# djeedai/bevy_hanabi

Hardware: AMD Instinct MI355X
Metric: particle-updates/sec (higher is better)
Workload: dtype f32

## Files before the change

### bevy_hanabi_amd/build.py

```python
import os
import subprocess
import sys
import sysconfig

_DIR = os.path.dirname(os.path.abspath(__file__))
_CSRC = os.path.join(_DIR, "csrc")

HIP_FLAGS = ["--offload-arch=gfx950", "-O3", "-std=c++17", "-ffp-contract=off", "-fhip-fp32-correctly-rounded-divide-sqrt",
             "-fPIC", "-shared", "-Wno-unused-value"]
HOST_FLAGS = ["-std=c++17", "-O2", "-fPIC", "-shared", "-ffp-contract=off", "-fvisibility=hidden"]


def _newer(target, sources):
    if not os.path.exists(target):
        return True
    t = os.path.getmtime(target)
    return any(os.path.getmtime(s) > t for s in sources)


def runtime_lib_path():
    return os.path.join(_DIR, "libhanabi_amd.so")


def host_module_path():
# ... 123 lines not shown
    return _build_code_object("hnb_import", "kImportCode", ["-ffp-contract=off"], force, verbose, headers=("hnb_import.h", "hnb_export.h", "hnb_export_rows.hip.h", "hnb_sort_key.h"))


IMPORT_CODE_OBJECTS = (build_import_code,)


def build_bounds_code(force=False, verbose=False):
    return _build_code_object("hnb_bounds", "kBoundsCode", ["-ffp-contract=off"], force, verbose, headers=("hnb_bounds.h", "hnb_sort_key.h"))


QUERY_CODE_OBJECTS = (build_bounds_code,)


def build_runtime(force=False, verbose=False):
    srcs = [os.path.join(_CSRC, "hanabi_amd.hip")] + sorted(os.path.join(_CSRC, f) for f in os.listdir(_CSRC) if f.endswith(".h"))
    srcs += [os.path.join(_DIR, "..", "include", h) for h in ("hanabi_amd.h", "hanabi_amd_binned.h", "hanabi_amd_import.h")]
    for build_code in EXPORT_CODE_OBJECTS + BINNED_CODE_OBJECTS + IMPORT_CODE_OBJECTS + QUERY_CODE_OBJECTS:
        srcs.append(build_code(force, verbose))
    out = runtime_lib_path()
    if force or _newer(out, srcs):
        embed_headers()
        hipcc = os.environ.get("HIPCC", "/opt/rocm/bin/hipcc")
        cmd = [hipcc] + HIP_FLAGS + [srcs[0], "-o", out, "-lhiprtc", "-ldl"]
        if verbose:
            print(" ".join(cmd))
        subprocess.check_call(cmd, cwd=_CSRC)
    return out


def build_host(force=False, verbose=False):
    import pybind11
# ... 63 lines not shown
```

### bevy_hanabi_amd/csrc/hanabi_amd.hip

```cpp
#include <hip/hip_runtime.h>

#include <algorithm>
#include <atomic>
#include <chrono>
#include <cmath>
#include <condition_variable>
#include <cstdarg>
#include <cstdio>
#include <cstring>
#include <deque>
#include <memory>
#include <mutex>
#include <string>
#include <thread>
#include <vector>

#include "hnb_kernels.hip.h"
#include "hnb_jit.h"
#include "hnb_sort.hip.h"
#include "hnb_comm.h"
#include "hnb_plan.h"
#include "hnb_program.h"
#include "hnb_export.h"
#include "hnb_export_code.inc"
#include "hnb_export_sort_code.inc"
#include "hnb_filter_pred.h"
#include "hnb_export_filter_code.inc"
#include "hnb_export_cull_code.inc"
#include "hnb_export_filter_prog_code.inc"
#include "hnb_export_cull_prog_code.inc"
#include "hnb_export_bin.h"
#include "hnb_export_bin_code.inc"
#include "hnb_import.h"
#include "hnb_import_code.inc"
#include "hnb_bounds.h"
#include "hnb_bounds_code.inc"

using namespace hnb;

namespace {

thread_local std::string g_last_error;

int fail(int code, const char* fmt, ...) {
    char buf[512];
    va_list ap;
    va_start(ap, fmt);
    vsnprintf(buf, sizeof buf, fmt, ap);
    va_end(ap);
    g_last_error = buf;
// ... 138 lines not shown
    bool direct_failed = false;
    uint64_t direct_frames = 0, copied_frames = 0;
    uint64_t ring_waits = 0, ring_wait_ns = 0;
    hipEvent_t stage_done[plan::kStageGroups] = {};
    plan::StageRing stage_ring;
    uint32_t num_cus = 256;
    std::vector<HnbProgram*> programs;
    HnbSimParams sim{};
    uint32_t frame = 0;
    uint32_t list_order = HNB_LIST_ORDER_SPAWN;
    ProgramOptions popt;
    bool skip_lists = true;
    bool alternate = true;
    bool suffix_proof = true;
    uint32_t slot_init = 1;
    bool ring_lists = true;
    bool scene_merge = true;
    bool transpose = true;
    uint32_t timing = 0;
    uint32_t timing_tick = 0;
    std::vector<TimingPair> t_update, t_init, t_compact;
    std::vector<hipEvent_t> event_pool;
    uint32_t comm_refs = 0;
    uint32_t set_mode = HNB_SET_MODULE_CACHED;
    struct SetModule {
        hipModule_t module = nullptr;
        hipFunction_t init = nullptr, update = nullptr;
        jit::SetPlan plan;
        uint32_t gen = 0;
    } set;
// ... 29 lines not shown
    uint32_t cull_dt_operand = 0;
    bool update_streams = false;
    uint32_t age_cohort_mode = HNB_AGE_COHORT_AUTO;
    bool auto_materialise = false;
    StreamLaunchFn stream_launch = nullptr;
    StreamLaunchFn stream_launch_fused = nullptr;
    uint32_t fuse_span = 1, fused_left = 0;
    uint32_t safe_launches = 0;
    std::vector<uint32_t> fuse_ublocks;
    uint32_t fused_frames = 0;
    const char* stream_kernel_name = "";
    hipModule_t jit_module = nullptr;
    hipFunction_t jit_init = nullptr, jit_update = nullptr, jit_init_slots = nullptr;
    bool slot_init_eligible = false;
    uint32_t slot_init_frames = 0;
    uint32_t sort_skipped_frames = 0;
    uint32_t sort_path_frames[3] = {0, 0, 0};
    bool tick_sign_seen = false;
    uint64_t serial = 0;
    bool jit_pending = false;
    std::string kernel_info, jit_log;
    enum class StepsState { NotRequested, Built, Pending, Failed };
    hipModule_t steps_module = nullptr;
    hipFunction_t steps_update = nullptr;
    StepsState steps_state = StepsState::NotRequested;
    bool steps_from_cache = false;
    std::string steps_why;
    std::vector<Ins> steps_ops;
    int steps_waves = 0;
    bool steps_cohort = false;
// ... 527 lines not shown
        case HNB_OPT_HORIZON: ctx->popt.horizon = value != 0u; return HNB_OK;
        case HNB_OPT_TEST_BREAK_PROOF: {
            const char* e = getenv("HNB_ENABLE_TEST_HOOKS");
            if (value != 0u && !(e && e[0] == '1')) return fail(HNB_ERR_INVALID_ARG, "HNB_OPT_TEST_BREAK_PROOF is a test hook: refused unless HNB_ENABLE_TEST_HOOKS=1 is set in the environment");
            ctx->break_proof = value != 0u;
            return HNB_OK;
        }
        case HNB_OPT_TRANSPOSE: ctx->transpose = value != 0u; return HNB_OK;
        case HNB_OPT_SCENE_MERGE: ctx->scene_merge = value != 0u; return HNB_OK;
        case HNB_OPT_SUFFIX_PROOF: ctx->suffix_proof = value != 0u; return HNB_OK;
        case HNB_OPT_RING_LISTS: ctx->ring_lists = value != 0u; return HNB_OK;
        case HNB_OPT_SLOT_INIT:
            if (value > 2u) return fail(HNB_ERR_INVALID_ARG, "unknown slot-init mode %u", value);
            ctx->slot_init = value;
            return HNB_OK;
        case HNB_OPT_STREAM_HINTS: ctx->stream_hints = value != 0u; return HNB_OK;
        case HNB_OPT_DIRECT_UPLOAD: ctx->direct_upload = value != 0u; return HNB_OK;
        case HNB_OPT_JIT_ASYNC: ctx->jit_async = value != 0u; return HNB_OK;
        case HNB_OPT_FUSE_STEPS: ctx->fuse_steps = value != 0u; return HNB_OK;
        case HNB_OPT_SET_MODULE:
            if (value > HNB_SET_MODULE_BACKGROUND) return fail(HNB_ERR_INVALID_ARG, "unknown set-module mode %u", value);
            ctx->set_mode = value;
            ctx->set_lookup = plan::SetLookupState();
            return HNB_OK;
        case HNB_OPT_OVERLAP_UPDATES: ctx->overlap_updates = value != 0u && ctx->side_stream && ctx->ev_fork && ctx->ev_join; return HNB_OK;
        default: return fail(HNB_ERR_INVALID_ARG, "unknown option %u", option);
    }
}

int hnb_ctx_synchronize(HnbContext* ctx) {
// ... 1031 lines not shown
        const uint32_t grid = split ? total_chunks * (kChunk / kBlock) : total_chunks;
        ctx->step_stats.update_launches += 1;
        if (p->jit_update) {
            uint32_t dm = write_died;
            void* ka[] = {&p->dev, &p->d_inst_base, &dfi, &dub, &cb, &dm, &split};
            HIP_TRY(hipModuleLaunchKernel(p->jit_update, grid, 1, 1, kBlock, 1, 1, 0, st, ka, nullptr));
        } else if (p->wide_file) k_update_slots_generic<InterpCodeWide><<<grid, kBlock, 0, st>>>(p->dev, p->d_inst_base, dfi, dub, cb, write_died, split);
        else k_update_slots_generic<InterpCode><<<grid, kBlock, 0, st>>>(p->dev, p->d_inst_base, dfi, dub, cb, write_died, split);
    }
    if (timed) { hipEventRecord(tu.b, st); ctx->t_update.push_back(tu); }
    const CompactArgs ca = compact_args_of(p);
    const bool lists = p->plan.lists;
    if (!lists) p->skipped_frames += p->fuse_span;
    else if (ca.suffix_dead) p->suffix_frames += 1;
    if (lists && p->dev.n_event_channels) {
        k_emit_count<<<total_chunks, kBlock, 0, st>>>(p->dev, p->d_inst_base, p->d_meta[par], dfi, cb);
        uint32_t max_ev = 0;
        for (const HnbEffect* fx : p->effects)
            for (const EventChannel& ch : fx->channels) max_ev = std::max(max_ev, ch.capacity);
        const uint32_t splits = plan::size_event_grid(max_ev, total_chunks);
        k_emit_events<<<dim3(total_chunks, splits), kBlock, 0, st>>>(p->dev, p->d_inst_base, p->d_meta[par], dfi, cb, p->h_ev_counts, ctx->frame);
    }
    if (!p->plan.lists_merged) {
        if (lists) ctx->step_stats.list_launches += ((!p->slot_order && !ca.suffix_dead) ? 2u : 1u) + (p->slot_order ? 2u : 0u);
        if (lists && !p->slot_order && !ca.suffix_dead) k_count_rows<<<total_chunks, kBlock, 0, st>>>(ca, p->d_inst_base, p->d_meta[par], dfi, cb);
        if (lists) k_compact<<<total_chunks, kBlock, 0, st>>>(ca, p->d_inst_base, p->d_meta[par], p->d_meta[par ^ 1], dfi, cb);
        if (lists && p->slot_order) {
            k_order_count<<<total_chunks, kBlock, 0, st>>>(ca, p->d_inst_base, p->d_meta[par], dfi, cb);
            k_order_write<<<total_chunks, kBlock, 0, st>>>(ca, p->d_inst_base, p->d_meta[par], p->d_meta[par ^ 1], dfi, cb);
        }
        if (timed) { tc.a = tu.b; hipEventRecord(tc.b, st); ctx->t_compact.push_back(tc); }
        if (p->has_ribbons) enqueue_ribbon_sort(ctx, p, st);
    }
    HIP_TRY(hipGetLastError());
    return HNB_OK;
}
// ... 925 lines not shown
        if (l.step == kImportStepMaterialise) { if ((rc = enqueue_export_materialise(p, fx->index, 1u)) != HNB_OK) return rc; }
        else if (l.step == kImportStepZeroCounts) HIP_TRY(hipMemsetAsync(d->out_count, 0, 8u, ctx->stream));
        else {
            void* ka[] = {&a};
            HIP_TRY(hipModuleLaunchKernel(ctx->import_fn[l.kernel], l.grid_x, 1, 1, kExportBlock, 1, 1, 0, ctx->stream, ka, nullptr));
        }
    }
    if (c.n_payload == 0u) return HNB_OK;
    return reset_plane_proofs(fx, c.has_age);
}
}

int hnb_effect_import(HnbEffect* fx, const HnbImportDesc* desc) {
    if (!fx || !desc) return fail(HNB_ERR_INVALID_ARG, "NULL argument");
    return run_import(fx, desc);
}

int hnb_program_export(HnbProgram* p, const HnbExportDesc* desc, uint32_t* out_offsets) {
    if (!p || !desc) return fail(HNB_ERR_INVALID_ARG, "NULL argument");
    return run_export(p, nullptr, desc, nullptr, nullptr, HNB_SORT_SCOPE_INSTANCE, out_offsets);
}

int hnb_program_export_sorted(HnbProgram* p, const HnbExportDesc* desc, const HnbExportSort* sort, uint32_t scope, uint32_t* out_offsets) {
    if (!p || !desc || !sort) return fail(HNB_ERR_INVALID_ARG, "NULL argument");
    if (scope > HNB_SORT_SCOPE_PROGRAM) return fail(HNB_ERR_INVALID_ARG, "scope %u: HNB_SORT_SCOPE_INSTANCE or HNB_SORT_SCOPE_PROGRAM", scope);
    if (scope == HNB_SORT_SCOPE_PROGRAM && out_offsets)
        return fail(HNB_ERR_INVALID_ARG, "out_offsets must be NULL with HNB_SORT_SCOPE_PROGRAM: the records are one order over all instances (tell them apart by an HNB_ATTR_ID field)");
    if (sort->struct_size == sizeof(HnbExportSortFiltered)) {
        if (scope == HNB_SORT_SCOPE_PROGRAM)
            return fail(HNB_ERR_INVALID_ARG, "an HnbExportSortFiltered takes HNB_SORT_SCOPE_INSTANCE: one order over all instances' kept rows (HNB_SORT_SCOPE_PROGRAM) is out of scope");
// ... 245 lines not shown
    }
    if (!prog->dev.age_cohort && prog->dev.cull_lifetime && prog->age_cohort_mode == HNB_AGE_COHORT_AUTO && (prog->hdr.render_reads_lo >> HNB_ATTR_AGE & 1u))
        s += "\nage cohorts: off (HNB_AGE_COHORT_AUTO: the asset's render modifiers read AGE after every frame)";
    if (prog->dev.age_cohort) {
        hipStreamSynchronize(prog->ctx->stream);
        std::vector<uint32_t> st(prog->dev.chunks_per_inst);
        size_t in_cohort = 0;
        for (const HnbEffect* fx : prog->effects) {
            if (hipMemcpy(st.data(), static_cast<const char*>(fx->slab) + prog->dev.lmin_off + (size_t)prog->dev.chunks_per_inst * 8, st.size() * 4, hipMemcpyDeviceToHost) != hipSuccess) break;
            for (uint32_t v : st) in_cohort += v == 1u ? 1u : 0u;
        }
        s += "\nage cohorts: " + std::to_string(in_cohort) + " of " + std::to_string(prog->effects.size() * (size_t)prog->dev.chunks_per_inst) + " chunks";
        if (prog->auto_materialise) s += " (HNB_AGE_COHORT_AUTO: the asset's render modifiers read AGE, the update keeps the plane current)";
    }
    if (prog->slot_init_frames) s += "\nslot-major init (large spawns): " + std::to_string(prog->slot_init_frames) + " frames";
    if (prog->has_ribbons && prog->suffix_frames) s += "\ncasualties proven to be the list's last rows (no k_count_rows): " + std::to_string(prog->suffix_frames) + " frames";
    if (prog->has_ribbons && prog->ring_frames) s += "\nlist kept as a ring (no row rewritten): " + std::to_string(prog->ring_frames) + " frames";
    if (prog->has_ribbons && prog->sort_skipped_frames) s += "\nribbon sorts skipped in list-free frames: " + std::to_string(prog->sort_skipped_frames) + " frames";
    if (prog->has_ribbons) s += "\nribbon sorts by rotation: " + std::to_string(prog->sort_rotated_frames) + " of " + std::to_string(prog->frames_run) + " frames" + (prog->ribbon_facts.front_static ? "" : " (not eligible)");
    if (prog->has_ribbons) s += "\nribbon sorts by path: one-tile " + std::to_string(prog->sort_path_frames[0]) + ", one-workgroup " + std::to_string(prog->sort_path_frames[1]) +
                                ", multi-launch " + std::to_string(prog->sort_path_frames[2]) + " frames";
    if (prog->merged_frames) s += "\nupdate served by a merged launch (small programs of the context share one): " + std::to_string(prog->merged_frames) + " frames";
    if (prog->unmerged_frames) s += "\nkept out of the shared launches (the loaded set module does not know this program; its own specialised kernels): " + std::to_string(prog->unmerged_frames) + " frames";
    if (prog->set_frames) s += "\n... by the context's set module (the program's specialised code behind the shared launch): " + std::to_string(prog->set_frames) + " frames";
    if (!prog->ctx->set_log.empty() && !prog->set_sig.empty()) s += "\nset module: " + prog->ctx->set_log;
    if (prog->ctx->set_failed_builds && !prog->set_sig.empty()) s += "\nset module builds that failed: " + std::to_string(prog->ctx->set_failed_builds);
    if (prog->horizon_eligible) s += "\ndeath horizons in use: " + std::to_string(prog->hz_frames) + " frames";
    s += "\nlists skipped: " + std::to_string(prog->skipped_frames) + " of " + std::to_string(prog->frames_run) + " frames" + (prog->skip_facts.eligible ? "" : " (not eligible)");
    s += "\nframe parameters (context): written by the host into device memory in " + std::to_string(prog->ctx->direct_frames) + " frames, copied in " + std::to_string(prog->ctx->copied_frames) +
         (prog->ctx->large_bar ? "" : " (the device memory is not host-visible: no large BAR)") + (prog->ctx->direct_failed ? " (host-visible slots failed their check)" : "");
// ... 270 lines not shown
```

### bevy_hanabi_amd/csrc/hnb_kernels.hip.h

```cpp
#pragma once
#ifndef __HIPCC_RTC__
#include <hip/hip_runtime.h>
#endif
#include "hnb_dev.h"

namespace hnb {

template <class T>
__device__ __forceinline__ T* global_ptr(uint64_t addr) {
    typedef __attribute__((address_space(1))) T global_t;
    return (T*)(global_t*)addr;
}

struct u2_t { uint32_t x, y; };
struct u3_t { uint32_t x, y, z; };
typedef uint32_t u4v __attribute__((ext_vector_type(4)));
#if defined(HNB_NONTEMPORAL) || defined(HNB_NONTEMPORAL_LOADS)
#define HNB_NT_LOAD(p) __builtin_nontemporal_load(p)
#else
#define HNB_NT_LOAD(p) (*(p))
#endif
#if defined(HNB_NONTEMPORAL) || defined(HNB_NONTEMPORAL_STORES)
#define HNB_NT_STORE(v, p) __builtin_nontemporal_store(v, p)
#else
// ... 875 lines not shown
        if (slot >= args.capacity) break;
        if (mask & (1u << b)) s_alive[pos++] = slot;
        else s_free[fpos++] = slot;
    }
    __syncthreads();
    uint32_t* list = reinterpret_cast<uint32_t*>(c.base + args.alive_off[meta_out[c.k].write_index & 1u]) + excl;
    for (uint32_t i = tid; i < chunk_alive; i += kBlock) list[i] = s_alive[i];
    const uint32_t alive_total = meta_out[c.k].alive_count;
    uint32_t* dead = reinterpret_cast<uint32_t*>(c.base + args.dead_off) + alive_total + (chunk_first - excl);
    for (uint32_t i = tid; i < chunk_slots - chunk_alive; i += kBlock) dead[i] = s_free[i];
}
#endif

#ifndef HNB_JIT_TU
constexpr uint32_t kEmitHeavy = 32u;
__global__ void __launch_bounds__(kBlock)
k_emit_events(const DevProgram prog, const uint64_t* __restrict__ inst_base, const DevMeta* __restrict__ meta_in,
              const DevFrameInst* __restrict__ fi, const CompactBufs cb, unsigned long long* __restrict__ ev_host, const uint32_t frame_tag) {
    __shared__ uint32_t s_red[kBlock / 64];
    __shared__ uint32_t s_scan[kBlock / 64];
    __shared__ uint32_t s_heavy_n;
    __shared__ uint32_t s_heavy[kChunk][3];
    const uint32_t tid = threadIdx.x, lane = tid & 63u, wave = tid >> 6;
    const uint32_t chunk = chunk_of_workgroup(cb.xcd_remap);
    const uint32_t split = blockIdx.y, n_split = gridDim.y;
    ChunkCtx c;
    const bool has_rows = chunk_setup(c, chunk, prog, inst_base, meta_in, fi);
    const bool last = c.n == 0 ? c.j == 0 : (c.start < c.n && c.start + kChunk >= c.n);
    const uint32_t rows = has_rows ? ((c.n - c.start) < kChunk ? (c.n - c.start) : kChunk) : 0u;
    constexpr uint32_t kPer = kChunk / kBlock;
    for (uint32_t ch = 0; ch < prog.n_event_channels; ++ch) {
        DevEventBuffer* ev = global_ptr<DevEventBuffer>(fi[c.k].ev_out[ch]);
        if (!ev) continue;
        const uint32_t* tot = cb.ev_totals + (size_t)c.k * prog.chunks_per_inst * HNB_MAX_EVENT_CHANNELS + ch;
        uint32_t part = 0;
        for (uint32_t i = tid; i < c.j; i += kBlock) part += tot[(size_t)i * HNB_MAX_EVENT_CHANNELS];
#pragma unroll
        for (uint32_t off = 32; off > 0; off >>= 1) part += __shfl_xor(part, off, 64);
        __syncthreads();
        if (lane == 0) s_red[wave] = part;
        if (tid == 0) s_heavy_n = 0u;
        __syncthreads();
        uint32_t excl = 0;
#pragma unroll
        for (uint32_t w = 0; w < kBlock / 64; ++w) excl += s_red[w];
        const uint32_t mine = has_rows ? tot[(size_t)c.j * HNB_MAX_EVENT_CHANNELS] : 0u;
        if (last && tid == 0 && split == 0u) {
            ev->count[fi[c.k].ev_parity] = excl + mine;
            if (ev_host) *reinterpret_cast<volatile unsigned long long*>(ev_host + (size_t)c.k * HNB_MAX_EVENT_CHANNELS + ch) = ((unsigned long long)(excl + mine) << 32) | frame_tag;
        }
        const uint32_t capacity = ev->capacity;
        if (mine == 0u || excl >= capacity) continue;
        const uint32_t* cnt = reinterpret_cast<const uint32_t*>(c.base + prog.ev_cnt_off[ch]);
        const uint32_t* slots = reinterpret_cast<const uint32_t*>(c.base + prog.alive_off[list_column(c.m.write_index)]) + c.start;
        uint32_t slot[kPer], n_ev[kPer], local = 0;
#pragma unroll
        for (uint32_t r = 0; r < kPer; ++r) {
            const uint32_t row = tid * kPer + r;
            slot[r] = row < rows ? slots[row] : 0u;
            n_ev[r] = row < rows ? cnt[slot[r]] : 0u;
            local += n_ev[r];
        }
        uint32_t incl = local;
#pragma unroll
        for (uint32_t off = 1; off < 64; off <<= 1) { const uint32_t y = __shfl_up(incl, off, 64); if (lane >= off) incl += y; }
        if (lane == 63) s_scan[wave] = incl;
        __syncthreads();
        uint32_t pos = excl + incl - local;
        for (uint32_t w = 0; w < wave; ++w) pos += s_scan[w];
#pragma unroll
        for (uint32_t r = 0; r < kPer; ++r) {
            if (n_ev[r] >= kEmitHeavy) {
                if ((tid * kPer + r) % n_split == split) {
                    const uint32_t h = atomicAdd(&s_heavy_n, 1u);
                    s_heavy[h][0] = slot[r]; s_heavy[h][1] = pos; s_heavy[h][2] = n_ev[r];
                }
            } else if (split == 0u) {
                const uint32_t end = pos + n_ev[r] < capacity ? pos + n_ev[r] : capacity;
                for (uint32_t e = pos; e < end; ++e) ev->data[e] = slot[r];
            }
            pos += n_ev[r];
        }
        __syncthreads();
        const uint32_t n_heavy = s_heavy_n;
        for (uint32_t h = 0; h < n_heavy; ++h) {
            const uint32_t sl = s_heavy[h][0], first = s_heavy[h][1];
            const uint32_t end = first + s_heavy[h][2] < capacity ? first + s_heavy[h][2] : capacity;
            for (uint32_t e = first + tid; e < end; e += kBlock) ev->data[e] = sl;
        }
        __syncthreads();
    }
}
#endif

#ifndef HNB_STREAM_WAVES
#define HNB_STREAM_WAVES 6
#endif
#ifndef HNB_STREAM_WAVES_FULL
#define HNB_STREAM_WAVES_FULL 5
#endif

template <bool B> struct BoolTag { static constexpr bool value = B; };
struct SlotArgs {
    uint32_t capacity, n_uregs, chunks_per_inst, n_inst;
    soff_t alive_flag_off;
    uint32_t update_len;
// ... 891 lines not shown
```

### bevy_hanabi_amd/csrc/hnb_plan.h

```cpp
#pragma once
#include <cstdint>
#include <cstring>

namespace hnb {
namespace plan {

struct InstanceFrame {
    bool simulated = true;
    bool has_parent = false;
    uint32_t spawn_count = 0;
    uint32_t event_capacity = 0;
    const uint32_t* ublock = nullptr;
};
inline uint32_t uword(const InstanceFrame& f, uint32_t decoded_operand) { return f.ublock[decoded_operand & 0xffu]; }
inline float as_float(uint32_t bits) { float f; std::memcpy(&f, &bits, 4); return f; }
inline bool nonneg_not_nan(uint32_t float_bits) { return float_bits <= 0x7f800000u; }

struct SkipFacts {
    bool eligible = false;
    uint32_t dt_operand = 0;
};
struct SkipHistory {
    double cum_tick[128] = {};
    uint32_t last_dirty = 0;
// ... 143 lines not shown
    if (in.has_parent && in.simulated) {
        request = in.event_capacity;
        if (in.events_known) request = in.known_events < in.event_capacity ? in.known_events : in.event_capacity;
    }
    const uint32_t capped = request < capacity ? request : capacity;
    uint32_t blocks = (uint32_t)(((uint64_t)capped + init_block - 1u) / init_block);
    if (big_burst) blocks = (blocks + rounds_if_big - 1u) / rounds_if_big;
    if (in.has_parent) blocks = blocks < num_cus * 8u ? blocks : num_cus * 8u;
    return blocks;
}
inline uint32_t size_event_grid(uint32_t max_event_capacity, uint32_t total_chunks) {
    const uint32_t per_chunk = max_event_capacity / (total_chunks ? total_chunks : 1u);
    const uint32_t splits = (per_chunk + 16383u) / 16384u;
    return splits < 1u ? 1u : (splits > 64u ? 64u : splits);
}

struct SlotInitDecision { bool use = false, marks = false; };
constexpr uint32_t kSlotInitMinChunks = 17;
inline SlotInitDecision plan_slot_init(bool eligible, uint32_t option, uint32_t capacity, uint32_t chunks_per_inst, const InstanceFrame* inst, uint32_t n) {
    SlotInitDecision d;
    if (!eligible || option == 0u || n == 0u || (option == 1u && (uint64_t)n * chunks_per_inst < kSlotInitMinChunks)) return d;
    uint64_t spawns = 0;
    bool partial = false;
    for (uint32_t i = 0; i < n; ++i) {
        if (inst[i].has_parent) return d;
        if (!inst[i].simulated || inst[i].spawn_count == 0u) continue;
        spawns += inst[i].spawn_count < capacity ? inst[i].spawn_count : capacity;
        partial = partial || inst[i].spawn_count < capacity;
    }
    d.use = spawns != 0u && (option >= 2u || spawns * 8u >= (uint64_t)n * capacity);
// ... 130 lines not shown
```

### bevy_hanabi_amd/runtime.py

```python
import ctypes as C
import os

import numpy as np

from . import build as _build

HNB_OK = 0
HNB_ERR_NO_DEVICE = -4
HNB_ERR_NOT_FOUND = -6

ATTR_COMPONENTS = [1, 1, 3, 3, 1, 1, 1, 4, 1, 1, 2, 3, 1, 1, 3, 3, 3, 1, 1, 1, 1, 1, 2, 2, 2, 2, 3, 3, 3, 3, 4, 4, 4, 4, 1, 1, 1, 1, 1]
ATTR_IS_FLOAT = [0, 0, 1, 1, 1, 1, 0, 1, 1, 1, 1, 1, 0, 0, 1, 1, 1, 0] + [1] * 16 + [0] * 5

ABI_SYMBOLS = [
    "hnb_last_error", "hnb_version", "hnb_ctx_create", "hnb_ctx_destroy", "hnb_ctx_set_stream", "hnb_ctx_synchronize",
    "hnb_program_create", "hnb_program_destroy", "hnb_program_validate", "hnb_effect_create", "hnb_effect_destroy",
    "hnb_effect_set_parent", "hnb_frame_begin", "hnb_effect_set_frame", "hnb_effect_set_property", "hnb_simulate",
    "hnb_effect_metadata", "hnb_effect_alive_count", "hnb_effect_read_attr", "hnb_effect_read_alive_list",
    "hnb_effect_read_dead_list", "hnb_effect_write_attr", "hnb_effect_sort_ribbons", "hnb_ctx_enable_kernel_timing",
    "hnb_ctx_kernel_timing", "hnb_program_kernel_info", "hnb_jit_precompile", "hnb_effect_set_simulated", "hnb_ctx_set_option", "hnb_program_set_frames", "hnb_effect_index",
    "hnb_ctx_profile_marker", "hnb_program_kernel_timing",
    "hnb_comm_create_local", "hnb_comm_unique_id", "hnb_comm_create_rank", "hnb_comm_allreduce_alive", "hnb_comm_destroy", "hnb_comm_set_library",
    "hnb_effect_device_view", "hnb_effect_materialise", "hnb_jit_precompile_set", "hnb_effect_check", "hnb_effect_compare", "hnb_comm_describe", "hnb_program_device_view",
    "hnb_simulate_steps", "hnb_effect_set_frames_ahead", "hnb_program_set_frames_ahead", "hnb_ctx_step_stats",
    "hnb_program_prepare_steps", "hnb_jit_precompile_steps",
    "hnb_effect_export", "hnb_program_export", "hnb_effect_export_sorted", "hnb_program_export_sorted",
    "hnb_effect_export_filtered", "hnb_effect_export_filtered_sorted", "hnb_program_export_filtered",
    "hnb_effect_bounds", "hnb_program_bounds",
]
ABI_BINNED_SYMBOLS = ["hnb_effect_export_binned"]
ABI_IMPORT_SYMBOLS = ["hnb_effect_import"]

OPTIONS = {"list_order": 1, "alternate": 2, "skip_lists": 3, "age_cohort": 4, "cull_lifetime": 5, "horizon": 6, "transpose": 7, "scene_merge": 8,
           "suffix_proof": 9, "overlap_updates": 10, "stream_hints": 11, "set_module": 12, "jit_async": 13, "test_break_proof": 15, "ring_lists": 16, "slot_init": 17, "direct_upload": 18, "fuse_steps": 19}
MAX_FUSED_STEPS = 8
SET_MODULE_OFF, SET_MODULE_CACHED, SET_MODULE_COMPILE, SET_MODULE_BACKGROUND = 0, 1, 2, 3


class HanabiError(RuntimeError):
    def __init__(self, code, message):
        super().__init__(f"[{code}] {message}")
        self.code = code


class SimParams(C.Structure):
    _fields_ = [("delta_time", C.c_float), ("time", C.c_float), ("virtual_delta_time", C.c_float), ("virtual_time", C.c_float),
                ("real_delta_time", C.c_float), ("real_time", C.c_float)]


# ... 279 lines not shown
        lib.hnb_program_set_frames_ahead.argtypes = [C.c_void_p, C.c_uint32, C.c_uint32, C.c_uint32, C.c_void_p, C.c_void_p, C.c_void_p]
        lib.hnb_ctx_step_stats.argtypes = [C.c_void_p, C.POINTER(StepStats)]
        lib.hnb_program_prepare_steps.argtypes = [C.c_void_p]
        lib.hnb_jit_precompile_steps.argtypes = [C.c_char_p, C.c_size_t]
        lib.hnb_effect_export.argtypes = [C.c_void_p, C.POINTER(ExportDesc)]
        lib.hnb_program_export.argtypes = [C.c_void_p, C.POINTER(ExportDesc), C.c_void_p]
        lib.hnb_effect_export_sorted.argtypes = [C.c_void_p, C.POINTER(ExportDesc), C.POINTER(ExportSort)]
        lib.hnb_program_export_sorted.argtypes = [C.c_void_p, C.POINTER(ExportDesc), C.POINTER(ExportSort), C.c_uint32, C.c_void_p]
        lib.hnb_effect_export_filtered.argtypes = [C.c_void_p, C.POINTER(ExportDesc), C.POINTER(ExportFilter)]
        lib.hnb_effect_export_filtered_sorted.argtypes = [C.c_void_p, C.POINTER(ExportDesc), C.POINTER(ExportFilter), C.POINTER(ExportSort)]
        lib.hnb_program_export_filtered.argtypes = [C.c_void_p, C.POINTER(ExportDesc), C.POINTER(ExportFilter), C.c_uint32, C.c_void_p]
        lib.hnb_effect_bounds.argtypes = [C.c_void_p, C.POINTER(BoundsDesc)]
        lib.hnb_program_bounds.argtypes = [C.c_void_p, C.POINTER(BoundsDesc)]
        lib.hnb_effect_export_binned.argtypes = [C.c_void_p, C.POINTER(ExportDesc), C.POINTER(ExportBins)]
        lib.hnb_effect_import.argtypes = [C.c_void_p, C.POINTER(ImportDesc)]
        _lib = lib
    return _lib


def _check(rc):
    if rc != HNB_OK:
        raise HanabiError(rc, load_library().hnb_last_error().decode())


def validate_program(blob: bytes):
    _check(load_library().hnb_program_validate(blob, len(blob)))


def jit_precompile(blob: bytes):
    _check(load_library().hnb_jit_precompile(blob, len(blob)))
# ... 240 lines not shown
            self._h = None
            self._prog._effects.remove(self)

    def index(self):
        out = C.c_uint32()
        _check(self._lib.hnb_effect_index(self._h, C.byref(out)))
        return out.value

    def set_simulated(self, simulated=True):
        _check(self._lib.hnb_effect_set_simulated(self._h, int(bool(simulated))))

    def set_parent(self, parent, channel, event_capacity=256):
        _check(self._lib.hnb_effect_set_parent(self._h, parent._h, int(channel), int(event_capacity)))
        self._parent = parent

    def set_frame(self, spawn_count, seed, transform=None):
        xf = None
        if transform is not None:
            xf = np.ascontiguousarray(np.asarray(transform, dtype=np.float32).reshape(12))
        _check(self._lib.hnb_effect_set_frame(self._h, int(spawn_count), int(seed) & 0xFFFFFFFF, None if xf is None else xf.ctypes.data))

    def set_frames_ahead(self, spawn_counts, seeds, transforms=None):
        sc = np.ascontiguousarray(spawn_counts, dtype=np.uint32)
        sd = np.ascontiguousarray(np.asarray(seeds, dtype=np.uint64) & 0xFFFFFFFF, dtype=np.uint32)
        assert sc.ndim == 1 and sc.shape == sd.shape
        xf = None if transforms is None else np.ascontiguousarray(transforms, dtype=np.float32).reshape(len(sc), 12)
        _check(self._lib.hnb_effect_set_frames_ahead(self._h, len(sc), sc.ctypes.data, sd.ctypes.data, None if xf is None else xf.ctypes.data))

    def set_property(self, name, values):
        v = np.atleast_1d(np.asarray(values))
# ... 97 lines not shown
```

### include/hanabi_amd.h

```cpp
#ifndef HANABI_AMD_H
#define HANABI_AMD_H

#ifndef __HIPCC_RTC__
#include <stddef.h>
#include <stdint.h>
#endif

#ifdef __cplusplus
extern "C" {
#endif

typedef enum HnbStatus {
    HNB_OK = 0,
    HNB_ERR_INVALID_ARG = -1,
    HNB_ERR_BAD_PROGRAM = -2,
    HNB_ERR_HIP = -3,
    HNB_ERR_NO_DEVICE = -4,
    HNB_ERR_OUT_OF_MEMORY = -5,
    HNB_ERR_NOT_FOUND = -6,
    HNB_ERR_DEVICE_FAULT = -7
} HnbStatus;

typedef enum HnbAttr {
    HNB_ATTR_ID = 0, HNB_ATTR_PARTICLE_COUNTER = 1,
// ... 162 lines not shown
#define HNB_LIST_ORDER_SLOT 1u
#define HNB_OPT_ALTERNATE 2u
#define HNB_OPT_SKIP_LISTS 3u
#define HNB_OPT_AGE_COHORT 4u
#define HNB_AGE_COHORT_OFF 0u
#define HNB_AGE_COHORT_LEAN 1u
#define HNB_AGE_COHORT_ALL 2u
#define HNB_AGE_COHORT_AUTO 3u
#define HNB_OPT_CULL_LIFETIME 5u
#define HNB_OPT_HORIZON 6u
#define HNB_OPT_TRANSPOSE 7u
#define HNB_OPT_SCENE_MERGE 8u
#define HNB_OPT_SUFFIX_PROOF 9u
#define HNB_OPT_RING_LISTS 16u
#define HNB_OPT_SLOT_INIT 17u
#define HNB_OPT_DIRECT_UPLOAD 18u
#define HNB_OPT_OVERLAP_UPDATES 10u
#define HNB_OPT_STREAM_HINTS 11u
#define HNB_OPT_JIT_ASYNC 13u
#define HNB_OPT_TEST_BREAK_PROOF 15u
#define HNB_OPT_SET_MODULE 12u
#define HNB_SET_MODULE_OFF 0u
#define HNB_SET_MODULE_CACHED 1u
#define HNB_SET_MODULE_COMPILE 2u
#define HNB_SET_MODULE_BACKGROUND 3u
#define HNB_OPT_FUSE_STEPS 19u
#define HNB_MAX_FUSED_STEPS 8u
int hnb_ctx_set_option(HnbContext* ctx, uint32_t option, uint32_t value);

int hnb_program_create(HnbContext* ctx, const void* blob, size_t blob_size, HnbProgram** out_prog);
// ... 222 lines not shown
```

Measured before the change: 125.2 billion.

## Fuse spawn-event count and emit into one kernel for small instances

Adds a templated k_emit_events that computes each chunk's exclusive event prefix itself. It rescans the earlier rows of the instance's alive list and sums their per-slot event counts across all channels at once, which removes the separate k_emit_count launch and its per-chunk totals. The fused path is used by default when an instance has at most 16 chunks. In exchange, each workgroup does redundant prefix reads that grow with its chunk position. The change also adds an hnb_effect_read_events API for reading event buffers.

```diff
diff --git a/bevy_hanabi_amd/build.py b/bevy_hanabi_amd/build.py
--- a/bevy_hanabi_amd/build.py
+++ b/bevy_hanabi_amd/build.py
@@ -161,7 +161,7 @@
 
 def build_runtime(force=False, verbose=False):
     srcs = [os.path.join(_CSRC, "hanabi_amd.hip")] + sorted(os.path.join(_CSRC, f) for f in os.listdir(_CSRC) if f.endswith(".h"))
-    srcs += [os.path.join(_DIR, "..", "include", h) for h in ("hanabi_amd.h", "hanabi_amd_binned.h", "hanabi_amd_import.h")]
+    srcs += [os.path.join(_DIR, "..", "include", h) for h in ("hanabi_amd.h", "hanabi_amd_binned.h", "hanabi_amd_import.h", "hanabi_amd_events.h")]
     for build_code in EXPORT_CODE_OBJECTS + BINNED_CODE_OBJECTS + IMPORT_CODE_OBJECTS + QUERY_CODE_OBJECTS:
         srcs.append(build_code(force, verbose))
     out = runtime_lib_path()
diff --git a/bevy_hanabi_amd/csrc/hanabi_amd.hip b/bevy_hanabi_amd/csrc/hanabi_amd.hip
--- a/bevy_hanabi_amd/csrc/hanabi_amd.hip
+++ b/bevy_hanabi_amd/csrc/hanabi_amd.hip
@@ -34,6 +34,7 @@
 #include "hnb_import.h"
 #include "hnb_import_code.inc"
 #include "hnb_bounds.h"
+#include "../../include/hanabi_amd_events.h"
 #include "hnb_bounds_code.inc"
 
 using namespace hnb;
@@ -202,6 +203,7 @@
     bool alternate = true;
     bool suffix_proof = true;
     uint32_t slot_init = 1;
+    uint32_t emit_fused = 1;
     bool ring_lists = true;
     bool scene_merge = true;
     bool transpose = true;
@@ -261,6 +263,7 @@
     hipFunction_t jit_init = nullptr, jit_update = nullptr, jit_init_slots = nullptr;
     bool slot_init_eligible = false;
     uint32_t slot_init_frames = 0;
+    uint32_t emit_fused_frames = 0, emit_pair_frames = 0;
     uint32_t sort_skipped_frames = 0;
     uint32_t sort_path_frames[3] = {0, 0, 0};
     bool tick_sign_seen = false;
@@ -818,6 +821,7 @@
             if (value > 2u) return fail(HNB_ERR_INVALID_ARG, "unknown slot-init mode %u", value);
             ctx->slot_init = value;
             return HNB_OK;
+        case HNB_OPT_EMIT_FUSED: ctx->emit_fused = value != 0u ? 1u : 0u; return HNB_OK;
         case HNB_OPT_STREAM_HINTS: ctx->stream_hints = value != 0u; return HNB_OK;
         case HNB_OPT_DIRECT_UPLOAD: ctx->direct_upload = value != 0u; return HNB_OK;
         case HNB_OPT_JIT_ASYNC: ctx->jit_async = value != 0u; return HNB_OK;
@@ -1879,12 +1883,19 @@
     if (!lists) p->skipped_frames += p->fuse_span;
     else if (ca.suffix_dead) p->suffix_frames += 1;
     if (lists && p->dev.n_event_channels) {
-        k_emit_count<<<total_chunks, kBlock, 0, st>>>(p->dev, p->d_inst_base, p->d_meta[par], dfi, cb);
         uint32_t max_ev = 0;
         for (const HnbEffect* fx : p->effects)
             for (const EventChannel& ch : fx->channels) max_ev = std::max(max_ev, ch.capacity);
         const uint32_t splits = plan::size_event_grid(max_ev, total_chunks);
-        k_emit_events<<<dim3(total_chunks, splits), kBlock, 0, st>>>(p->dev, p->d_inst_base, p->d_meta[par], dfi, cb, p->h_ev_counts, ctx->frame);
+        if (plan::use_emit_fused(ctx->emit_fused, p->dev.chunks_per_inst)) {
+            if (p->dev.n_event_channels <= 2u) k_emit_events<2><<<dim3(total_chunks, splits), kBlock, 0, st>>>(p->dev, p->d_inst_base, p->d_meta[par], dfi, cb, p->h_ev_counts, ctx->frame);
+            else k_emit_events<HNB_MAX_EVENT_CHANNELS><<<dim3(total_chunks, splits), kBlock, 0, st>>>(p->dev, p->d_inst_base, p->d_meta[par], dfi, cb, p->h_ev_counts, ctx->frame);
+            p->emit_fused_frames += 1;
+        } else {
+            k_emit_count<<<total_chunks, kBlock, 0, st>>>(p->dev, p->d_inst_base, p->d_meta[par], dfi, cb);
+            k_emit_events<<<dim3(total_chunks, splits), kBlock, 0, st>>>(p->dev, p->d_inst_base, p->d_meta[par], dfi, cb, p->h_ev_counts, ctx->frame);
+            p->emit_pair_frames += 1;
+        }
     }
     if (!p->plan.lists_merged) {
         if (lists) ctx->step_stats.list_launches += ((!p->slot_order && !ca.suffix_dead) ? 2u : 1u) + (p->slot_order ? 2u : 0u);
@@ -2840,6 +2851,23 @@
 int hnb_effect_import(HnbEffect* fx, const HnbImportDesc* desc) {
     if (!fx || !desc) return fail(HNB_ERR_INVALID_ARG, "NULL argument");
     return run_import(fx, desc);
+}
+
+int hnb_effect_read_events(HnbEffect* parent, uint32_t channel, uint32_t* out_count, uint32_t* dst, uint32_t dst_capacity) {
+    if (!parent || !out_count || (!dst && dst_capacity)) return fail(HNB_ERR_INVALID_ARG, "NULL argument");
+    if (channel >= HNB_MAX_EVENT_CHANNELS) return fail(HNB_ERR_INVALID_ARG, "channel %u: at most %u event channels", channel, HNB_MAX_EVENT_CHANNELS);
+    const EventChannel& ch = parent->channels[channel];
+    if (!ch.buf) return fail(HNB_ERR_NOT_FOUND, "nobody listens on channel %u of this effect", channel);
+    HnbContext* ctx = parent->prog->ctx;
+    HIP_TRY(hipSetDevice(ctx->device));
+    HIP_TRY(hipStreamSynchronize(ctx->stream));
+    uint32_t head[4] = {};
+    HIP_TRY(hipMemcpy(head, ch.buf, sizeof head, hipMemcpyDeviceToHost));
+    const uint32_t count = ctx->frame ? head[(ctx->frame - 1u) & 1u] : 0u;
+    *out_count = count;
+    const uint32_t n = std::min(std::min(count, ch.capacity), dst_capacity);
+    if (n) HIP_TRY(hipMemcpy(dst, reinterpret_cast<const char*>(ch.buf) + offsetof(DevEventBuffer, data), (size_t)n * 4, hipMemcpyDeviceToHost));
+    return HNB_OK;
 }
 
 int hnb_program_export(HnbProgram* p, const HnbExportDesc* desc, uint32_t* out_offsets) {
@@ -3115,6 +3143,7 @@
         if (prog->auto_materialise) s += " (HNB_AGE_COHORT_AUTO: the asset's render modifiers read AGE, the update keeps the plane current)";
     }
     if (prog->slot_init_frames) s += "\nslot-major init (large spawns): " + std::to_string(prog->slot_init_frames) + " frames";
+    if (prog->emit_pair_frames) s += "\nspawn events ordered by k_emit_count + k_emit_events (two launches): " + std::to_string(prog->emit_pair_frames) + " of " + std::to_string(prog->emit_pair_frames + prog->emit_fused_frames) + " emitting frames";
     if (prog->has_ribbons && prog->suffix_frames) s += "\ncasualties proven to be the list's last rows (no k_count_rows): " + std::to_string(prog->suffix_frames) + " frames";
     if (prog->has_ribbons && prog->ring_frames) s += "\nlist kept as a ring (no row rewritten): " + std::to_string(prog->ring_frames) + " frames";
     if (prog->has_ribbons && prog->sort_skipped_frames) s += "\nribbon sorts skipped in list-free frames: " + std::to_string(prog->sort_skipped_frames) + " frames";
diff --git a/bevy_hanabi_amd/csrc/hnb_kernels.hip.h b/bevy_hanabi_amd/csrc/hnb_kernels.hip.h
--- a/bevy_hanabi_amd/csrc/hnb_kernels.hip.h
+++ b/bevy_hanabi_amd/csrc/hnb_kernels.hip.h
@@ -913,13 +913,76 @@
 
 #ifndef HNB_JIT_TU
 constexpr uint32_t kEmitHeavy = 32u;
+constexpr uint32_t kEmitPer = kChunk / kBlock;
+constexpr uint32_t kEmitNone = 0xffffffffu;
+struct EmitLds {
+    uint32_t* scan;
+    uint32_t* heavy_n;
+    uint32_t* heavy;
+};
+__device__ __forceinline__ uint32_t emit_store_rows(const EmitLds& lds, DevEventBuffer* ev, const uint32_t capacity, const uint32_t excl,
+                                                    const uint32_t (&slot)[kEmitPer], const uint32_t (&n_ev)[kEmitPer], const uint32_t split, const uint32_t n_split) {
+    const uint32_t tid = threadIdx.x, lane = tid & 63u, wave = tid >> 6;
+    uint32_t local = 0;
+#pragma unroll
+    for (uint32_t r = 0; r < kEmitPer; ++r) local += n_ev[r];
+    uint32_t incl = local;
+#pragma unroll
+    for (uint32_t off = 1; off < 64; off <<= 1) { const uint32_t y = __shfl_up(incl, off, 64); if (lane >= off) incl += y; }
+    if (lane == 63) lds.scan[wave] = incl;
+    if (tid == 0) *lds.heavy_n = 0u;
+    __syncthreads();
+    const uint32_t first = [&] { uint32_t p = excl + incl - local; for (uint32_t w = 0; w < wave; ++w) p += lds.scan[w]; return p; }();
+    uint32_t total = 0;
+#pragma unroll
+    for (uint32_t w = 0; w < kBlock / 64; ++w) total += lds.scan[w];
+    if (total == 0u || excl >= capacity) { __syncthreads(); return total; }
+    {
+        uint32_t pos = first;
+#pragma unroll
+        for (uint32_t r = 0; r < kEmitPer; ++r) {
+            if (n_ev[r] >= kEmitHeavy && (tid * kEmitPer + r) % n_split == split) {
+                const uint32_t h = atomicAdd(lds.heavy_n, 1u);
+                lds.heavy[h * 3u] = slot[r]; lds.heavy[h * 3u + 1u] = pos; lds.heavy[h * 3u + 2u] = n_ev[r];
+            }
+            pos += n_ev[r];
+        }
+    }
+    __syncthreads();
+    const uint32_t n_heavy = *lds.heavy_n;
+    if (split == 0u) {
+        const uint32_t w_end = capacity - excl < total ? capacity : excl + total;
+        uint32_t p = first;
+#pragma unroll
+        for (uint32_t r = 0; r < kEmitPer; ++r) {
+            if (n_ev[r] < kEmitHeavy) {
+                const uint32_t end = p + n_ev[r] < w_end ? p + n_ev[r] : w_end;
+                for (uint32_t e = p; e < end; ++e) ev->data[e] = slot[r];
+            }
+            p += n_ev[r];
+        }
+    }
+    for (uint32_t h = 0; h < n_heavy; ++h) {
+        const uint32_t sl = lds.heavy[h * 3u], hf = lds.heavy[h * 3u + 1u];
+        const uint32_t end = hf + lds.heavy[h * 3u + 2u] < capacity ? hf + lds.heavy[h * 3u + 2u] : capacity;
+        for (uint32_t e = hf + tid; e < end; e += kBlock) ev->data[e] = sl;
+    }
+    __syncthreads();
+    return total;
+}
+__device__ __forceinline__ void emit_publish_count(DevEventBuffer* ev, uint32_t parity, uint32_t count, unsigned long long* ev_host, uint32_t k, uint32_t ch, uint32_t frame_tag) {
+    ev->count[parity] = count;
+    if (ev_host) *reinterpret_cast<volatile unsigned long long*>(ev_host + (size_t)k * HNB_MAX_EVENT_CHANNELS + ch) = ((unsigned long long)count << 32) | frame_tag;
+}
+
 __global__ void __launch_bounds__(kBlock)
 k_emit_events(const DevProgram prog, const uint64_t* __restrict__ inst_base, const DevMeta* __restrict__ meta_in,
               const DevFrameInst* __restrict__ fi, const CompactBufs cb, unsigned long long* __restrict__ ev_host, const uint32_t frame_tag) {
     __shared__ uint32_t s_red[kBlock / 64];
     __shared__ uint32_t s_scan[kBlock / 64];
     __shared__ uint32_t s_heavy_n;
-    __shared__ uint32_t s_heavy[kChunk][3];
+    __shared__ uint32_t s_heavy[kChunk * 3u];
+    const EmitLds lds{s_scan, &s_heavy_n, s_heavy};
     const uint32_t tid = threadIdx.x, lane = tid & 63u, wave = tid >> 6;
     const uint32_t chunk = chunk_of_workgroup(cb.xcd_remap);
     const uint32_t split = blockIdx.y, n_split = gridDim.y;
@@ -927,7 +990,6 @@
     const bool has_rows = chunk_setup(c, chunk, prog, inst_base, meta_in, fi);
     const bool last = c.n == 0 ? c.j == 0 : (c.start < c.n && c.start + kChunk >= c.n);
     const uint32_t rows = has_rows ? ((c.n - c.start) < kChunk ? (c.n - c.start) : kChunk) : 0u;
-    constexpr uint32_t kPer = kChunk / kBlock;
     for (uint32_t ch = 0; ch < prog.n_event_channels; ++ch) {
         DevEventBuffer* ev = global_ptr<DevEventBuffer>(fi[c.k].ev_out[ch]);
         if (!ev) continue;
@@ -936,59 +998,119 @@
         for (uint32_t i = tid; i < c.j; i += kBlock) part += tot[(size_t)i * HNB_MAX_EVENT_CHANNELS];
 #pragma unroll
         for (uint32_t off = 32; off > 0; off >>= 1) part += __shfl_xor(part, off, 64);
-        __syncthreads();
         if (lane == 0) s_red[wave] = part;
-        if (tid == 0) s_heavy_n = 0u;
         __syncthreads();
         uint32_t excl = 0;
 #pragma unroll
         for (uint32_t w = 0; w < kBlock / 64; ++w) excl += s_red[w];
+        __syncthreads();
         const uint32_t mine = has_rows ? tot[(size_t)c.j * HNB_MAX_EVENT_CHANNELS] : 0u;
-        if (last && tid == 0 && split == 0u) {
-            ev->count[fi[c.k].ev_parity] = excl + mine;
-            if (ev_host) *reinterpret_cast<volatile unsigned long long*>(ev_host + (size_t)c.k * HNB_MAX_EVENT_CHANNELS + ch) = ((unsigned long long)(excl + mine) << 32) | frame_tag;
-        }
+        if (last && tid == 0 && split == 0u) emit_publish_count(ev, fi[c.k].ev_parity, excl + mine, ev_host, c.k, ch, frame_tag);
         const uint32_t capacity = ev->capacity;
         if (mine == 0u || excl >= capacity) continue;
         const uint32_t* cnt = reinterpret_cast<const uint32_t*>(c.base + prog.ev_cnt_off[ch]);
         const uint32_t* slots = reinterpret_cast<const uint32_t*>(c.base + prog.alive_off[list_column(c.m.write_index)]) + c.start;
-        uint32_t slot[kPer], n_ev[kPer], local = 0;
-#pragma unroll
-        for (uint32_t r = 0; r < kPer; ++r) {
-            const uint32_t row = tid * kPer + r;
+        uint32_t slot[kEmitPer], n_ev[kEmitPer];
+#pragma unroll
+        for (uint32_t r = 0; r < kEmitPer; ++r) {
+            const uint32_t row = tid * kEmitPer + r;
             slot[r] = row < rows ? slots[row] : 0u;
             n_ev[r] = row < rows ? cnt[slot[r]] : 0u;
-            local += n_ev[r];
-        }
-        uint32_t incl = local;
-#pragma unroll
-        for (uint32_t off = 1; off < 64; off <<= 1) { const uint32_t y = __shfl_up(incl, off, 64); if (lane >= off) incl += y; }
-        if (lane == 63) s_scan[wave] = incl;
-        __syncthreads();
-        uint32_t pos = excl + incl - local;
-        for (uint32_t w = 0; w < wave; ++w) pos += s_scan[w];
-#pragma unroll
-        for (uint32_t r = 0; r < kPer; ++r) {
-            if (n_ev[r] >= kEmitHeavy) {
-                if ((tid * kPer + r) % n_split == split) {
-                    const uint32_t h = atomicAdd(&s_heavy_n, 1u);
-                    s_heavy[h][0] = slot[r]; s_heavy[h][1] = pos; s_heavy[h][2] = n_ev[r];
-                }
-            } else if (split == 0u) {
-                const uint32_t end = pos + n_ev[r] < capacity ? pos + n_ev[r] : capacity;
-                for (uint32_t e = pos; e < end; ++e) ev->data[e] = slot[r];
-            }
-            pos += n_ev[r];
-        }
-        __syncthreads();
-        const uint32_t n_heavy = s_heavy_n;
-        for (uint32_t h = 0; h < n_heavy; ++h) {
-            const uint32_t sl = s_heavy[h][0], first = s_heavy[h][1];
-            const uint32_t end = first + s_heavy[h][2] < capacity ? first + s_heavy[h][2] : capacity;
-            for (uint32_t e = first + tid; e < end; e += kBlock) ev->data[e] = sl;
-        }
-        __syncthreads();
-    }
+        }
+        emit_store_rows(lds, ev, capacity, excl, slot, n_ev, split, n_split);
+    }
+}
+
+template <uint32_t NCH>
+__device__ __forceinline__ void emit_fused_chunk(const EmitLds& lds, const DevProgram& prog, const uint64_t* __restrict__ inst_base, const DevMeta* __restrict__ meta_in,
+                                                 const DevFrameInst* __restrict__ fi, const CompactBufs& cb, unsigned long long* __restrict__ ev_host, const uint32_t frame_tag) {
+    constexpr uint32_t kBatch = NCH <= 2u ? 32u : 16u;
+    constexpr bool kLoadAll = NCH <= 2u;
+    const uint32_t tid = threadIdx.x, lane = tid & 63u, wave = tid >> 6;
+    const uint32_t chunk = chunk_of_workgroup(cb.xcd_remap);
+    const uint32_t split = blockIdx.y, n_split = gridDim.y;
+    const uint32_t n_ch = prog.n_event_channels < NCH ? prog.n_event_channels : NCH;
+    const uint32_t k = chunk / prog.chunks_per_inst;
+    DevEventBuffer* ev[NCH];
+#pragma unroll
+    for (uint32_t ch = 0; ch < NCH; ++ch) ev[ch] = ch < n_ch ? global_ptr<DevEventBuffer>(fi[k].ev_out[ch]) : nullptr;
+    const uint32_t parity = fi[k].ev_parity;
+    ChunkCtx c;
+    const bool has_rows = chunk_setup(c, chunk, prog, inst_base, meta_in, fi);
+    const bool last = c.n == 0 ? c.j == 0 : (c.start < c.n && c.start + kChunk >= c.n);
+    if (!has_rows && !last) return;
+    uint32_t capacity[NCH];
+#pragma unroll
+    for (uint32_t ch = 0; ch < NCH; ++ch) capacity[ch] = ev[ch] ? ev[ch]->capacity : 0u;
+    const uint32_t rows = has_rows ? ((c.n - c.start) < kChunk ? (c.n - c.start) : kChunk) : 0u;
+    const uint32_t* list = reinterpret_cast<const uint32_t*>(c.base + prog.alive_off[list_column(c.m.write_index)]);
+    uint32_t slot[kEmitPer], n_ev[NCH][kEmitPer];
+#pragma unroll
+    for (uint32_t r = 0; r < kEmitPer; ++r) { const uint32_t row = tid * kEmitPer + r; slot[r] = row < rows ? list[c.start + row] : kEmitNone; }
+#pragma unroll
+    for (uint32_t ch = 0; ch < NCH; ++ch) pin_scalar(capacity[ch]);
+#pragma unroll
+    for (uint32_t ch = 0; ch < NCH; ++ch) {
+        const uint32_t* cnt = reinterpret_cast<const uint32_t*>(c.base + prog.ev_cnt_off[ch < n_ch ? ch : 0u]);
+#pragma unroll
+        for (uint32_t r = 0; r < kEmitPer; ++r) n_ev[ch][r] = 0u;
+        if (kLoadAll || ev[ch]) {
+#pragma unroll
+            for (uint32_t r = 0; r < kEmitPer; ++r) { const uint32_t v = cnt[slot[r] != kEmitNone ? slot[r] : 0u]; n_ev[ch][r] = (ev[ch] && slot[r] != kEmitNone) ? v : 0u; }
+        }
+    }
+    uint32_t acc[NCH];
+#pragma unroll
+    for (uint32_t ch = 0; ch < NCH; ++ch) acc[ch] = 0u;
+    for (uint32_t b = 0; b < c.start; b += kBatch * kBlock) {
+        uint32_t s[kBatch];
+#pragma unroll
+        for (uint32_t q = 0; q < kBatch; ++q) { const uint32_t row = b + q * kBlock + tid; s[q] = row < c.start ? list[row] : kEmitNone; }
+#pragma unroll
+        for (uint32_t ch = 0; ch < NCH; ++ch) {
+            const uint32_t* cnt = reinterpret_cast<const uint32_t*>(c.base + prog.ev_cnt_off[ch < n_ch ? ch : 0u]);
+            if (kLoadAll || ev[ch]) {
+                uint32_t g[kBatch];
+#pragma unroll
+                for (uint32_t q = 0; q < kBatch; ++q) g[q] = cnt[s[q] != kEmitNone ? s[q] : 0u];
+#pragma unroll
+                for (uint32_t q = 0; q < kBatch; ++q) acc[ch] += s[q] != kEmitNone ? g[q] : 0u;
+            }
+        }
+    }
+#pragma unroll
+    for (uint32_t ch = 0; ch < NCH; ++ch) {
+#pragma unroll
+        for (uint32_t off = 32; off > 0; off >>= 1) acc[ch] += __shfl_xor(acc[ch], off, 64);
+        if (lane == 0) lds.heavy[ch * (kBlock / 64) + wave] = acc[ch];
+    }
+    __syncthreads();
+    uint32_t excl[NCH];
+#pragma unroll
+    for (uint32_t ch = 0; ch < NCH; ++ch) {
+        excl[ch] = 0u;
+#pragma unroll
+        for (uint32_t w = 0; w < kBlock / 64; ++w) excl[ch] += lds.heavy[ch * (kBlock / 64) + w];
+    }
+    __syncthreads();
+#pragma unroll
+    for (uint32_t r = 0; r < kEmitPer; ++r) slot[r] = slot[r] == kEmitNone ? 0u : slot[r];
+#pragma unroll
+    for (uint32_t ch = 0; ch < NCH; ++ch) {
+        if (!ev[ch]) continue;
+        const uint32_t total = emit_store_rows(lds, ev[ch], capacity[ch], excl[ch], slot, n_ev[ch], split, n_split);
+        if (last && tid == 0 && split == 0u) emit_publish_count(ev[ch], parity, excl[ch] + total, ev_host, c.k, ch, frame_tag);
+    }
+}
+template <uint32_t NCH>
+__global__ void __launch_bounds__(kBlock)
+k_emit_events(const DevProgram prog, const uint64_t* __restrict__ inst_base, const DevMeta* __restrict__ meta_in,
+              const DevFrameInst* __restrict__ fi, const CompactBufs cb, unsigned long long* __restrict__ ev_host, const uint32_t frame_tag) {
+    __shared__ uint32_t s_scan[kBlock / 64];
+    __shared__ uint32_t s_heavy_n;
+    __shared__ uint32_t s_heavy[kChunk * 3u];
+    static_assert(NCH * (kBlock / 64) <= kChunk * 3u, "the prefix words fit the heavy queue");
+    emit_fused_chunk<NCH>(EmitLds{s_scan, &s_heavy_n, s_heavy}, prog, inst_base, meta_in, fi, cb, ev_host, frame_tag);
 }
 #endif
 
diff --git a/bevy_hanabi_amd/csrc/hnb_plan.h b/bevy_hanabi_amd/csrc/hnb_plan.h
--- a/bevy_hanabi_amd/csrc/hnb_plan.h
+++ b/bevy_hanabi_amd/csrc/hnb_plan.h
@@ -181,6 +181,8 @@
     const uint32_t splits = (per_chunk + 16383u) / 16384u;
     return splits < 1u ? 1u : (splits > 64u ? 64u : splits);
 }
+constexpr uint32_t kEmitFusedChunks = 16;
+inline bool use_emit_fused(uint32_t option, uint32_t chunks_per_inst) { return option != 0u && chunks_per_inst >= 1u && chunks_per_inst <= kEmitFusedChunks; }
 
 struct SlotInitDecision { bool use = false, marks = false; };
 constexpr uint32_t kSlotInitMinChunks = 17;
diff --git a/bevy_hanabi_amd/runtime.py b/bevy_hanabi_amd/runtime.py
--- a/bevy_hanabi_amd/runtime.py
+++ b/bevy_hanabi_amd/runtime.py
@@ -30,9 +30,10 @@
 ]
 ABI_BINNED_SYMBOLS = ["hnb_effect_export_binned"]
 ABI_IMPORT_SYMBOLS = ["hnb_effect_import"]
+ABI_EVENTS_SYMBOLS = ["hnb_effect_read_events"]
 
 OPTIONS = {"list_order": 1, "alternate": 2, "skip_lists": 3, "age_cohort": 4, "cull_lifetime": 5, "horizon": 6, "transpose": 7, "scene_merge": 8,
-           "suffix_proof": 9, "overlap_updates": 10, "stream_hints": 11, "set_module": 12, "jit_async": 13, "test_break_proof": 15, "ring_lists": 16, "slot_init": 17, "direct_upload": 18, "fuse_steps": 19}
+           "suffix_proof": 9, "overlap_updates": 10, "stream_hints": 11, "set_module": 12, "jit_async": 13, "test_break_proof": 15, "ring_lists": 16, "slot_init": 17, "direct_upload": 18, "fuse_steps": 19, "emit_fused": 20}
 MAX_FUSED_STEPS = 8
 SET_MODULE_OFF, SET_MODULE_CACHED, SET_MODULE_COMPILE, SET_MODULE_BACKGROUND = 0, 1, 2, 3
 
@@ -342,6 +343,7 @@
         lib.hnb_program_bounds.argtypes = [C.c_void_p, C.POINTER(BoundsDesc)]
         lib.hnb_effect_export_binned.argtypes = [C.c_void_p, C.POINTER(ExportDesc), C.POINTER(ExportBins)]
         lib.hnb_effect_import.argtypes = [C.c_void_p, C.POINTER(ImportDesc)]
+        lib.hnb_effect_read_events.argtypes = [C.c_void_p, C.c_uint32, C.POINTER(C.c_uint32), C.c_void_p, C.c_uint32]
         _lib = lib
     return _lib
 
@@ -612,6 +614,12 @@
         _check(self._lib.hnb_effect_set_parent(self._h, parent._h, int(channel), int(event_capacity)))
         self._parent = parent
 
+    def read_events(self, channel, max_events):
+        n = C.c_uint32()
+        out = np.zeros(max(int(max_events), 1), dtype=np.uint32)
+        _check(self._lib.hnb_effect_read_events(self._h, int(channel), C.byref(n), out.ctypes.data, int(max_events)))
+        return int(n.value), out[:min(int(n.value), int(max_events))]
+
     def set_frame(self, spawn_count, seed, transform=None):
         xf = None
         if transform is not None:
diff --git a/include/hanabi_amd.h b/include/hanabi_amd.h
--- a/include/hanabi_amd.h
+++ b/include/hanabi_amd.h
@@ -200,6 +200,7 @@
 #define HNB_OPT_SUFFIX_PROOF 9u
 #define HNB_OPT_RING_LISTS 16u
 #define HNB_OPT_SLOT_INIT 17u
+#define HNB_OPT_EMIT_FUSED 20u
 #define HNB_OPT_DIRECT_UPLOAD 18u
 #define HNB_OPT_OVERLAP_UPDATES 10u
 #define HNB_OPT_STREAM_HINTS 11u
diff --git a/include/hanabi_amd_events.h b/include/hanabi_amd_events.h
--- /dev/null
+++ b/include/hanabi_amd_events.h
@@ -0,0 +1,15 @@
+#ifndef HANABI_AMD_EVENTS_H
+#define HANABI_AMD_EVENTS_H
+
+#include "hanabi_amd.h"
+
+#ifdef __cplusplus
+extern "C" {
+#endif
+
+int hnb_effect_read_events(HnbEffect* parent, uint32_t channel, uint32_t* out_count, uint32_t* dst, uint32_t dst_capacity);
+
+#ifdef __cplusplus
+}
+#endif
+#endif
```

Result: no change. 125.1 billion (-0.1%).
